# sanweiliti/RoHM

Measured on AMD Instinct MI355X. Metric: denoised 145-frame clips/sec @1000 DDPM steps, higher is better.
Workload: dtype f32

## Files before the change

rohm_amd/csrc/attention_tile.h:

```cpp
#pragma once
#include "common.h"
#include "planes.h"

namespace rohm {

constexpr int AT_S = 144;
constexpr int AT_DH = 128;
constexpr int AT_NB = 9;
constexpr int AT_TILE = AT_S * AT_DH;
constexpr int AT_LDS_FLOATS = 2 * AT_TILE + 512;

#define AT_WAIT_VM(n) __builtin_amdgcn_s_waitcnt(((n) & 15) | (7 << 4) | (15 << 8) | (((n) >> 4) << 14))
#define AT_WAIT_LGKM0() __builtin_amdgcn_s_waitcnt(15 | (7 << 4) | (0 << 8) | (3 << 14))

template <int AUX>
__device__ __forceinline__ void at_dma16(const float* src, float* lds_dst) {
    __builtin_amdgcn_global_load_lds((const __attribute__((address_space(1))) void*)src,
                                     (__attribute__((address_space(3))) void*)lds_dst, 16, 0, AUX);
}

#ifdef AT_TIMELINE
#define AT_TL_PARAM , unsigned long long* __restrict__ tl
#define AT_STAMP(i)                                                                                          \
    do {                                                                                                     \
        if (lane == 0) tl[((size_t)blockIdx.x * NW + wave) * 16 + (i)] = __builtin_amdgcn_s_memtime();     \
    } while (0)
#else
#define AT_TL_PARAM
#define AT_STAMP(i)
#endif

template <int NW, int NPO = 0, int AUX = 0, int NPASS = 1>
__device__ __forceinline__ void attention_item(const float* __restrict__ qkv, float* __restrict__ ctx, int n_head, int item, int q0,
                                               int nq, float* smem, const int tid AT_TL_PARAM) {
    constexpr int OWNED = NW * NPASS;
    constexpr int NQP = (NPASS == 2) ? 72 / NW : ((NW == 8) ? 9 : 10);
    constexpr int NKP = 24 / NW;
    constexpr int NVP = 72 / NW;
    constexpr int NV3 = NVP / 3;
    constexpr int NT = (AT_NB + NW - 1) / NW;
    float* Ks = smem;
    float* Vs = smem + AT_TILE;
    float* dummy = smem + 2 * AT_TILE;
    float* stats = dummy + 256;

    const int lane = tid & 63;
    const int wave = __builtin_amdgcn_readfirstlane(tid >> 6);
    const int li = lane & 15, lg = lane >> 4;

    AT_STAMP(0);
    const bool coop = nq > OWNED;
    const int seq = item / n_head, head = item % n_head;
    const int D = n_head * AT_DH;
    const size_t ldq = (size_t)3 * D;
    const float* qg = qkv + (size_t)seq * AT_S * ldq + head * AT_DH;
    const float* kg = qg + D;
    const float* vg = qg + 2 * D;

    const int half_row = lane >> 5, cphys = lane & 31;
#pragma unroll
    for (int i = 0; i < NQP; ++i) {
        const int lp = i * NW + wave;
        const bool ok = lp < nq * 8;
        const int lr = ok ? 2 * lp + half_row : half_row;
        const float* src = qg + (size_t)(q0 * 16 + lr) * ldq + ((cphys ^ (lr & 15)) << 2);
        at_dma16<AUX>(src, ok ? Vs + lp * 256 : dummy);
    }
    auto issue_k = [&](int G) {
#pragma unroll
        for (int i = 0; i < NKP; ++i) {
            const int piece = 24 * G + i * NW + wave;
            const int row = 2 * piece + half_row;
            at_dma16<AUX>(kg + (size_t)row * ldq + ((cphys ^ (row & 15)) << 2), Ks + piece * 256);
        }
    };
    issue_k(0);
    AT_WAIT_VM(NKP);
    __builtin_amdgcn_s_barrier();
    AT_STAMP(1);

    f32x4 qf[NPASS][8], qc[8];
#pragma unroll
    for (int ks = 0; ks < 8; ++ks) {
#pragma unroll
        for (int ps = 0; ps < NPASS; ++ps)
            qf[ps][ks] = *reinterpret_cast<const f32x4*>(Vs + ((ps * NW + wave) * 16 + li) * AT_DH + (((ks * 4 + lg) ^ li) << 2));
        qc[ks] = *reinterpret_cast<const f32x4*>(Vs + ((coop ? OWNED : 0) * 16 + li) * AT_DH + (((ks * 4 + lg) ^ li) << 2));
    }
    AT_WAIT_LGKM0();
    __builtin_amdgcn_s_barrier();
    auto issue_v = [&](int part) {
#pragma unroll
        for (int i = part * NV3; i < (part + 1) * NV3; ++i) {
            const int piece = i * NW + wave;
            at_dma16<AUX>(vg + (size_t)(2 * piece + half_row) * ldq + (cphys << 2), Vs + piece * 256);
        }
    };
    issue_k(1);
    issue_k(2);

    f32x4 sacc[NPASS][AT_NB];
#pragma unroll
    for (int ps = 0; ps < NPASS; ++ps)
#pragma unroll
        for (int kb = 0; kb < AT_NB; ++kb) sacc[ps][kb] = f32x4{0.f, 0.f, 0.f, 0.f};
#pragma unroll
    for (int G = 0; G < 3; ++G) {
        if (G == 0) {
            AT_WAIT_VM(2 * NKP);
        } else if (G == 1) {
            issue_v(0);
            issue_v(1);
            AT_WAIT_VM(NKP + 2 * NV3);
        } else {
            issue_v(2);
            AT_WAIT_VM(3 * NV3);
        }
        __builtin_amdgcn_s_barrier();
        AT_STAMP(2 + G);
        auto kread = [&](f32x4* kf, int ks) {
#pragma unroll
            for (int c = 0; c < 3; ++c)
                kf[c] = *reinterpret_cast<const f32x4*>(Ks + ((3 * G + c) * 16 + li) * AT_DH + (((ks * 4 + lg) ^ li) << 2));
        };
        f32x4 kf[2][3];
        kread(kf[0], 0);
#pragma unroll
        for (int ks = 0; ks < 8; ++ks) {
#pragma unroll
            for (int c = 0; c < 3; ++c)
                sacc[0][3 * G + c] = __builtin_amdgcn_mfma_f32_16x16x4f32(kf[ks & 1][c][0], qf[0][ks][0], sacc[0][3 * G + c], 0, 0, 0);
            __builtin_amdgcn_sched_barrier(0);
            if (ks + 1 < 8) kread(kf[(ks + 1) & 1], ks + 1);
            __builtin_amdgcn_sched_barrier(0);
#pragma unroll
            for (int j = 1; j < 4; ++j)
#pragma unroll
                for (int c = 0; c < 3; ++c)
                    sacc[0][3 * G + c] = __builtin_amdgcn_mfma_f32_16x16x4f32(kf[ks & 1][c][j], qf[0][ks][j], sacc[0][3 * G + c], 0, 0, 0);
        }
    }
    if constexpr (NPASS == 2) {
#pragma unroll
        for (int G = 0; G < 3; ++G) {
            auto kread = [&](f32x4* kf, int ks) {
#pragma unroll
                for (int c = 0; c < 3; ++c)
                    kf[c] = *reinterpret_cast<const f32x4*>(Ks + ((3 * G + c) * 16 + li) * AT_DH + (((ks * 4 + lg) ^ li) << 2));
            };
            f32x4 kf[2][3];
            kread(kf[0], 0);
#pragma unroll
            for (int ks = 0; ks < 8; ++ks) {
#pragma unroll
                for (int c = 0; c < 3; ++c)
                    sacc[NPASS - 1][3 * G + c] = __builtin_amdgcn_mfma_f32_16x16x4f32(kf[ks & 1][c][0], qf[NPASS - 1][ks][0], sacc[NPASS - 1][3 * G + c], 0, 0, 0);
                __builtin_amdgcn_sched_barrier(0);
                if (ks + 1 < 8) kread(kf[(ks + 1) & 1], ks + 1);
                __builtin_amdgcn_sched_barrier(0);
#pragma unroll
                for (int j = 1; j < 4; ++j)
#pragma unroll
                    for (int c = 0; c < 3; ++c)
                        sacc[NPASS - 1][3 * G + c] = __builtin_amdgcn_mfma_f32_16x16x4f32(kf[ks & 1][c][j], qf[NPASS - 1][ks][j], sacc[NPASS - 1][3 * G + c], 0, 0, 0);
            }
        }
    }
    f32x4 cs[NT];
#pragma unroll
    for (int t = 0; t < NT; ++t) cs[t] = f32x4{0.f, 0.f, 0.f, 0.f};
    if (coop) {
// ... 15 lines not shown
    AT_STAMP(5);
    constexpr float LOG2E = 1.4426950408889634f;
#pragma unroll
    for (int ps = 0; ps < NPASS; ++ps) {
        float mx = sacc[ps][0][0];
#pragma unroll
        for (int kb = 0; kb < AT_NB; ++kb)
#pragma unroll
            for (int r = 0; r < 4; ++r) mx = fmaxf(mx, sacc[ps][kb][r]);
        mx = fmaxf(mx, __shfl_xor(mx, 16));
        mx = fmaxf(mx, __shfl_xor(mx, 32));
        const float mb = mx * LOG2E;
        float sum = 0.f;
#pragma unroll
        for (int kb = 0; kb < AT_NB; ++kb)
#pragma unroll
            for (int r = 0; r < 4; ++r) {
                const float e = __builtin_amdgcn_exp2f(fmaf(sacc[ps][kb][r], LOG2E, -mb));
                sacc[ps][kb][r] = e;
                sum += e;
            }
        sum += __shfl_xor(sum, 16);
        sum += __shfl_xor(sum, 32);
        const float inv = 1.0f / sum;
#pragma unroll
        for (int kb = 0; kb < AT_NB; ++kb)
#pragma unroll
            for (int r = 0; r < 4; ++r) sacc[ps][kb][r] *= inv;
    }
    float c_m = -INFINITY, c_l = 0.f;
    if (coop) {
#pragma unroll
        for (int t = 0; t < NT; ++t)
            if (wave + t * NW < AT_NB)
#pragma unroll
                for (int r = 0; r < 4; ++r) c_m = fmaxf(c_m, cs[t][r]);
        c_m = fmaxf(c_m, __shfl_xor(c_m, 16));
        c_m = fmaxf(c_m, __shfl_xor(c_m, 32));
        const float mb = c_m * LOG2E;
#pragma unroll
        for (int t = 0; t < NT; ++t)
            if (wave + t * NW < AT_NB)
#pragma unroll
                for (int r = 0; r < 4; ++r) {
                    const float e = __builtin_amdgcn_exp2f(fmaf(cs[t][r], LOG2E, -mb));
                    cs[t][r] = e;
                    c_l += e;
                }
        c_l += __shfl_xor(c_l, 16);
        c_l += __shfl_xor(c_l, 32);
    }

    AT_STAMP(6);
    AT_WAIT_VM(0);
    __builtin_amdgcn_s_barrier();
    AT_STAMP(7);

    if (coop) {
        float* part = Ks + wave * (16 * AT_DH);
#pragma unroll
        for (int db = 0; db < 2; ++db) {
            f32x4 oacc[4];
#pragma unroll
            for (int m = 0; m < 4; ++m) oacc[m] = f32x4{0.f, 0.f, 0.f, 0.f};
#pragma unroll
            for (int t = 0; t < NT; ++t) {
                const int kb = wave + t * NW;
                if (kb < AT_NB) {
#pragma unroll
                    for (int j = 0; j < 4; ++j) {
                        const f32x4 vf = *reinterpret_cast<const f32x4*>(Vs + (kb * 16 + lg * 4 + j) * AT_DH + db * 64 + li * 4);
#pragma unroll
                        for (int m = 0; m < 4; ++m)
                            oacc[m] = __builtin_amdgcn_mfma_f32_16x16x4f32(cs[t][j], vf[m], oacc[m], 0, 0, 0);
                    }
                }
            }
#pragma unroll
            for (int r = 0; r < 4; ++r)
                *reinterpret_cast<f32x4*>(part + (lg * 4 + r) * AT_DH + db * 64 + li * 4) =
                    f32x4{oacc[0][r], oacc[1][r], oacc[2][r], oacc[3][r]};
        }
        if (lg == 0) {
            stats[(wave * 16 + li) * 2 + 0] = c_m;
            stats[(wave * 16 + li) * 2 + 1] = c_l;
        }
    }
    AT_STAMP(9);

    {
        auto pv_mfma = [](float pval, float vval, const f32x4& c) {
            if constexpr (NPO == 0) return __builtin_amdgcn_mfma_f32_16x16x4f32(pval, vval, c, 0, 0, 0);
            else return __builtin_amdgcn_mfma_f32_16x16x4f32(vval, pval, c, 0, 0, 0);
        };
#pragma unroll
        for (int ps = 0; ps < NPASS; ++ps) {
        float* out = ctx + ((size_t)seq * AT_S + (q0 + ps * NW + wave) * 16) * D + head * AT_DH;
#pragma unroll
        for (int db = 0; db < 2; ++db) {
            f32x4 oacc[4];
#pragma unroll
            for (int m = 0; m < 4; ++m) oacc[m] = f32x4{0.f, 0.f, 0.f, 0.f};
            auto vread = [&](int st) {
                return *reinterpret_cast<const f32x4*>(Vs + ((st >> 2) * 16 + lg * 4 + (st & 3)) * AT_DH + db * 64 + li * 4);
            };
            f32x4 vf[2][2];
            vf[0][0] = vread(0);
            vf[0][1] = vread(1);
#pragma unroll
            for (int sp = 0; sp < 2 * AT_NB; ++sp) {
                const int st = 2 * sp;
                oacc[0] = pv_mfma(sacc[ps][st >> 2][st & 3], vf[sp & 1][0][0], oacc[0]);
                __builtin_amdgcn_sched_barrier(0);
                if (sp + 1 < 2 * AT_NB) {
                    vf[(sp + 1) & 1][0] = vread(st + 2);
                    vf[(sp + 1) & 1][1] = vread(st + 3);
                }
                __builtin_amdgcn_sched_barrier(0);
#pragma unroll
                for (int m = 1; m < 4; ++m)
                    oacc[m] = pv_mfma(sacc[ps][st >> 2][st & 3], vf[sp & 1][0][m], oacc[m]);
#pragma unroll
                for (int m = 0; m < 4; ++m)
                    oacc[m] = pv_mfma(sacc[ps][(st + 1) >> 2][(st + 1) & 3], vf[sp & 1][1][m], oacc[m]);
            }
            if constexpr (NPO == 0) {
#pragma unroll
                for (int r = 0; r < 4; ++r)
                    *reinterpret_cast<f32x4*>(out + (size_t)(lg * 4 + r) * D + db * 64 + li * 4) =
                        f32x4{oacc[0][r], oacc[1][r], oacc[2][r], oacc[3][r]};
            } else {
                const int row = seq * AT_S + (q0 + ps * NW + wave) * 16 + li;
                const int kg0 = (head * AT_DH + db * 64 + lg * 16) >> 3;
#pragma unroll
                for (int h = 0; h < 2; ++h)
                    plane_store8<(NPO ? NPO : 2)>(reinterpret_cast<char*>(ctx), row, kg0 + h, D / 32,
                                                  f32x4{oacc[0][2 * h], oacc[1][2 * h], oacc[2][2 * h], oacc[3][2 * h]},
                                                  f32x4{oacc[0][2 * h + 1], oacc[1][2 * h + 1], oacc[2][2 * h + 1], oacc[3][2 * h + 1]});
            }
        }
        }
    }
    AT_STAMP(8);
    if (!coop) return;

    AT_WAIT_LGKM0();
    __builtin_amdgcn_s_barrier();
    AT_STAMP(10);
    {
        float* out = ctx + ((size_t)seq * AT_S + (q0 + OWNED) * 16) * D + head * AT_DH;
        for (int u = tid; u < 16 * 32; u += NW * 64) {
            const int q = u >> 5, c4 = u & 31;
            float M = -INFINITY;
#pragma unroll
            for (int w = 0; w < NW; ++w) M = fmaxf(M, stats[(w * 16 + q) * 2]);
            float e[NW], L = 0.f;
#pragma unroll
// ... 24 lines not shown
```

rohm_amd/csrc/encoder_chain.hip:

```cpp
#include <type_traits>
#include "common.h"
#include "gemm_sched.h"
#include "attention_tile.h"

namespace rohm {

typedef float f32x16c __attribute__((ext_vector_type(16)));

namespace chain {

constexpr int BM = 144, BK = kGemmBK, NRB = BM / 16;
constexpr int A_UNITS = BM * 8, A_ITERS = (A_UNITS + 255) / 256;
constexpr int kMaxBN = 384;
constexpr int kZone = 2 * (BM + kMaxBN) * BK;
constexpr int kLdsFloats = kZone + 512 + 4 * BM * 2;
constexpr int kSc1 = 16;

struct PhaseArgs {
    const float* A; int lda;
    const float* W; int ldw;
    float* C; int ldc;
    int K;
    const float* bias;
    const float* R; int ldr;
    const float* gamma; const float* beta; float eps; int ln_dim;
    int qcols; float qscale;
    int S; const float* tab; const float* tab0; int ldtab, ldtab0, tab_by_row;
    int m0, n0;
    float* row_stats; unsigned tag28; int tn, tiles_n;
    unsigned* err; unsigned xcc1; int fault;
};

template <int BN>
__device__ __forceinline__ void prefetch_w(const float* W, int ldw, int n0, float* smem, int tid, int wave_u) {
    constexpr int B_ITERS = BN * 8 / 256;
    float* Bs = smem + 2 * BM * BK;
#pragma unroll
    for (int buf = 0; buf < 2; ++buf)
#pragma unroll
        for (int i = 0; i < B_ITERS; ++i) {
            const int u = tid + i * 256;
            const int row = u >> 3;
            const int slot = (u & 7) ^ ((row >> 1) & 7);
            const float* src = W + (size_t)(n0 + row) * ldw + slot * 4 + buf * BK;
            __builtin_amdgcn_global_load_lds((const __attribute__((address_space(1))) void*)src,
                                             (__attribute__((address_space(3))) void*)(Bs + buf * (BN * BK) + (i * 256 + wave_u) * 4), 16, 0, 0);
        }
}

__device__ __forceinline__ void group_sync(unsigned long long* flags, int tn, int G, unsigned tag, unsigned xcc1, unsigned* err, int tid) {
    asm volatile("s_waitcnt vmcnt(0)" ::: "memory");
    __syncthreads();
    if (tid == 0) {
        flags[tn] = ((unsigned long long)xcc1 << 32) | tag;
        asm volatile("" ::: "memory");
    }
    if (tid < G && tid != tn) {
        for (int it = 0;; ++it) {
            const unsigned long long f = __hip_atomic_load(flags + tid, __ATOMIC_RELAXED, __HIP_MEMORY_SCOPE_AGENT);
            if ((unsigned)f == tag && (f >> 32) != 0ull) {
                if ((unsigned)(f >> 32) != xcc1) __hip_atomic_store(err, 2u, __ATOMIC_RELAXED, __HIP_MEMORY_SCOPE_AGENT);
                break;
            }
            __builtin_amdgcn_s_sleep(1);
            if ((it & 127) == 127 && __hip_atomic_load(err, __ATOMIC_RELAXED, __HIP_MEMORY_SCOPE_AGENT) != 0u) break;
            if (it > (1 << 19)) {
                __hip_atomic_store(err, 1u, __ATOMIC_RELAXED, __HIP_MEMORY_SCOPE_AGENT);
                break;
            }
        }
    }
    __syncthreads();
}

template <int BN, int EPI, bool PREF, bool SC1, bool REFETCH, typename AfterLoop>
__device__ __forceinline__ void gemm_phase(const PhaseArgs& p, float* smem, const int tid, AfterLoop&& after_loop) {
    static_assert(EPI == EPI_BIAS_RES_LN || EPI == EPI_BIAS_GELU || EPI == EPI_QKV || EPI == EPI_EMBED, "chain phases: LN tail, GELU, QKV, embed");
    constexpr int WN = BN / 4;
    constexpr int NCB = WN / 16;
    constexpr int B_ITERS = BN * 8 / 256;
    constexpr int PIECES = A_ITERS + B_ITERS;
    constexpr int AUX = SC1 ? kSc1 : 0;

    float* As = smem;
    float* Bs = smem + 2 * BM * BK;
    float* lds_dummy = smem + kZone;
    float* const zone = lds_dummy + 512;

    const int lane = tid & 63;
    const int wave = tid >> 6;
    const int li = lane & 15, lg = lane >> 4;
    const int wave_u = __builtin_amdgcn_readfirstlane(wave) * 64;
    const int m0 = p.m0, n0 = p.n0;

    const float* a_src[A_ITERS];
#pragma unroll
    for (int i = 0; i < A_ITERS; ++i) {
        const int u = tid + i * 256;
        const int row = (u < A_UNITS) ? (u >> 3) : 0;
        const int slot = (u & 7) ^ ((row >> 1) & 7);
        a_src[i] = p.A + (size_t)(m0 + row) * p.lda + slot * 4;
    }
    const float* b_src[B_ITERS];
#pragma unroll
    for (int i = 0; i < B_ITERS; ++i) {
        const int u = tid + i * 256;
        const int row = u >> 3;
        const int slot = (u & 7) ^ ((row >> 1) & 7);
        b_src[i] = p.W + (size_t)(n0 + row) * p.ldw + slot * 4;
    }
    auto dma_a = [&](int buf, int k0) {
#pragma unroll
        for (int piece = 0; piece < A_ITERS; ++piece) {
            float* dst = As + buf * (BM * BK) + (piece * 256 + wave_u) * 4;
            if (piece == A_ITERS - 1 && A_UNITS % 256 != 0)
                dst = (wave_u < A_UNITS - (A_ITERS - 1) * 256) ? dst : lds_dummy + (wave_u & 64) * 4;
            __builtin_amdgcn_global_load_lds((const __attribute__((address_space(1))) void*)(a_src[piece] + k0),
                                             (__attribute__((address_space(3))) void*)dst, 16, 0, AUX);
        }
    };
    auto dma_b = [&](int buf, int k0) {
#pragma unroll
        for (int i = 0; i < B_ITERS; ++i)
            __builtin_amdgcn_global_load_lds((const __attribute__((address_space(1))) void*)(b_src[i] + k0),
                                             (__attribute__((address_space(3))) void*)(Bs + buf * (BN * BK) + (i * 256 + wave_u) * 4), 16, 0, 0);
    };

    f32x4 acc16[NRB * NCB];
#pragma unroll
    for (int i = 0; i < NRB * NCB; ++i) acc16[i] = f32x4{0.f, 0.f, 0.f, 0.f};
    constexpr int READS = NRB + NCB;
    constexpr int MFMAS = 4 * NRB * NCB;
    struct Frag { f32x4 a[NRB]; f32x4 b[NCB]; };
    Frag f0, f1;
    auto read_frags = [&](Frag& f, int buf, int ks) {
        const float* as = As + buf * (BM * BK);
        const float* bs = Bs + buf * (BN * BK) + wave * WN * BK;
        const int slot = ks * 4 + lg;
#pragma unroll
        for (int c = 0; c < NCB; ++c) f.b[c] = *reinterpret_cast<const f32x4*>(bs + lds_off(c * 16 + li, slot));
#pragma unroll
        for (int r = 0; r < NRB; ++r) f.a[r] = *reinterpret_cast<const f32x4*>(as + lds_off(r * 16 + li, slot));
    };
    auto mma_half = [&](const Frag& f) {
#pragma unroll
        for (int r = 0; r < NRB; ++r)
#pragma unroll
            for (int c = 0; c < NCB; ++c)
#pragma unroll
                for (int j = 0; j < 4; ++j)
                    acc16[r * NCB + c] = __builtin_amdgcn_mfma_f32_16x16x4f32(f.b[c][j], f.a[r][j], acc16[r * NCB + c], 0, 0, 0);
    };

    const int nk = p.K / BK;
    constexpr bool COL_LDS = BN >= 384;
    if constexpr (!PREF) { dma_b(0, 0); dma_b(1, BK); }
    if constexpr (COL_LDS) {
        if (wave == 0) {
#pragma unroll
            for (int h = 0; h < 2; ++h) {
                const int unit = h * 64 + lane;
                const float* src = p.bias + n0 + (unit < BN / 4 ? unit : BN / 4 - 1) * 4;
                __builtin_amdgcn_global_load_lds((const __attribute__((address_space(1))) void*)src,
                                                 (__attribute__((address_space(3))) void*)(zone + h * 256), 16, 0, 0);
            }
        }
    }
    dma_a(0, 0);
    dma_a(1, BK);

    const int nw = n0 + wave * WN;
    struct ColOps { f32x4 bias, g4, b4; };
    constexpr bool RES = (EPI == EPI_BIAS_RES_LN);
    constexpr bool HAS_RES = RES || EPI == EPI_EMBED;
    constexpr bool PEEL = BN <= 256;
    constexpr bool EARLY = PEEL && !COL_LDS;
    const f32x4 zero4 = f32x4{0.f, 0.f, 0.f, 0.f};
    auto load_col = [&](int nb) __attribute__((always_inline)) {
        ColOps o{zero4, zero4, zero4};
        if constexpr (EPI == EPI_EMBED) {  }
        else if constexpr (COL_LDS) o.bias = *reinterpret_cast<const f32x4*>(zone + (nb - n0));
        else o.bias = *reinterpret_cast<const f32x4*>(p.bias + nb);
        if constexpr (RES) {
            o.g4 = *reinterpret_cast<const f32x4*>(p.gamma + nb);
            o.b4 = *reinterpret_cast<const f32x4*>(p.beta + nb);
        }
        return o;
    };
    auto for_units = [&](auto&& fn) __attribute__((always_inline)) {
#pragma unroll
        for (int r = 0; r < NRB; ++r)
#pragma unroll
            for (int c = 0; c < NCB; ++c) fn(c * NRB + r, c, m0 + r * 16 + li, nw + c * 16 + lg * 4, acc16[r * NCB + c]);
    };
    ColOps col[NCB];
    f32x4 res[HAS_RES ? NCB * NRB : 1];
    auto request_ops = [&]() __attribute__((always_inline)) {
#pragma unroll
        for (int c = 0; c < NCB; ++c) col[c] = load_col(nw + c * 16 + lg * 4);
        if constexpr (RES)
            for_units([&](int i, int, int m, int nb, f32x4) __attribute__((always_inline)) {
                res[i] = *reinterpret_cast<const f32x4*>(p.R + (size_t)m * p.ldr + nb);
            });
        if constexpr (EPI == EPI_EMBED)
            for_units([&](int i, int, int m, int nb, f32x4) __attribute__((always_inline)) {
                const int bidx = m / p.S, tok = m % p.S;
                const float* tp = (tok == 0) ? p.tab0 + (size_t)bidx * p.ldtab0 + nb : p.tab + (size_t)(p.tab_by_row ? m : tok) * p.ldtab + nb;
                res[i] = *reinterpret_cast<const f32x4*>(tp);
            });
    };

    asm volatile("s_waitcnt vmcnt(%0)" ::"n"(A_ITERS) : "memory");
    __syncthreads();
    read_frags(f0, 0, 0);
    constexpr int NG = READS;
    constexpr int MF = (MFMAS + NG - 1) / NG;
    auto chunk = [&](int kc, auto last_tag, auto dma_tag) __attribute__((always_inline)) {
        constexpr bool LAST = decltype(last_tag)::value;
        constexpr bool DMA = decltype(dma_tag)::value;
        const int buf = kc & 1;
        if constexpr (LAST && EARLY) request_ops();
        read_frags(f1, buf, 1);
        mma_half(f0);
        SchedGroups<0, NG, MF, READS, 0, 0>::run();
        __builtin_amdgcn_sched_barrier(0);
        if constexpr (!LAST) {
            asm volatile("s_waitcnt vmcnt(0)" ::: "memory");
            __syncthreads();
            __builtin_amdgcn_sched_barrier(0);
            if constexpr (DMA) {
                const int kn = ((kc + 2 < nk) ? (kc + 2) : (nk - 1)) * BK;
                dma_a(buf, kn);
                dma_b(buf, kn);
            }
// ... 93 lines not shown
                    }
                }
                bool ok = true, same_xcd = true;
#pragma unroll
                for (int k = 0; k < 8; ++k) {
                    mk[k] = 0.f; qk[k] = 0.f;
                    if (k >= tiles_n) continue;
                    if (k == tn) { mk[k] = a; qk[k] = b; continue; }
                    const unsigned tl = (unsigned)(lo[k] >> 32), th = (unsigned)(hi[k] >> 32);
                    ok = ok && (tl >> 4) == ep28 && (th >> 4) == ep28 && (tl & 15u) != 0u && (th & 15u) != 0u;
                    same_xcd = same_xcd && (tl & 15u) == xcc1 && (th & 15u) == xcc1;
                    mk[k] = __uint_as_float((unsigned)lo[k]);
                    qk[k] = __uint_as_float((unsigned)hi[k]);
                }
                if (ok) {
                    if (!same_xcd) __hip_atomic_store(p.err, 2u, __ATOMIC_RELAXED, __HIP_MEMORY_SCOPE_AGENT);
                    break;
                }
                __builtin_amdgcn_s_sleep(1);
                if ((it & 127) == 127 && __hip_atomic_load(p.err, __ATOMIC_RELAXED, __HIP_MEMORY_SCOPE_AGENT) != 0u) break;
                if (it > (1 << 19)) {
                    __hip_atomic_store(p.err, 1u, __ATOMIC_RELAXED, __HIP_MEMORY_SCOPE_AGENT);
                    break;
                }
            }
            constexpr float kT = (float)BN;
            if (tiles_n > 1) {
                merge(mk[0], qk[0], mk[1], qk[1], kT, mk[0], qk[0]);
                if (tiles_n > 2) merge(mk[2], qk[2], mk[3], qk[3], kT, mk[2], qk[2]);
                if (tiles_n > 4) { merge(mk[4], qk[4], mk[5], qk[5], kT, mk[4], qk[4]); merge(mk[6], qk[6], mk[7], qk[7], kT, mk[6], qk[6]); }
            }
            if (tiles_n > 2) {
                merge(mk[0], qk[0], mk[2], qk[2], 2.0f * kT, mk[0], qk[0]);
                if (tiles_n > 4) merge(mk[4], qk[4], mk[6], qk[6], 2.0f * kT, mk[4], qk[4]);
            }
            if (tiles_n > 4) merge(mk[0], qk[0], mk[4], qk[4], 4.0f * kT, mk[0], qk[0]);
            const float mu = mk[0];
            const float var = qk[0] / (float)p.ln_dim;
            *reinterpret_cast<f32x2*>(part + tid * 2) = f32x2{mu, 1.0f / sqrtf(var + p.eps)};
        }
        __syncthreads();
#pragma unroll
        for (int r = 0; r < NRB; ++r) {
            const f32x2 mrv = *reinterpret_cast<const f32x2*>(part + (r * 16 + li) * 2);
#pragma unroll
            for (int c = 0; c < NCB; ++c) {
                const f32x4 a = acc16[r * NCB + c];
                f32x4 v;
#pragma unroll
                for (int q = 0; q < 4; ++q) v[q] = (a[q] - mrv[0]) * mrv[1] * col[c].g4[q] + col[c].b4[q];
                *reinterpret_cast<f32x4*>(p.C + (size_t)(m0 + r * 16 + li) * p.ldc + nw + c * 16 + lg * 4) = v;
            }
        }
    } else if constexpr (EPI == EPI_EMBED) {
        for_units([&](int i, int, int m, int nb, f32x4 a) __attribute__((always_inline)) {
            const int tok = m % p.S;
            f32x4 v;
#pragma unroll
            for (int q = 0; q < 4; ++q) v[q] = (tok == 0 ? 0.f : a[q]) + res[i][q];
            *reinterpret_cast<f32x4*>(p.C + (size_t)m * p.ldc + nb) = v;
        });
    } else {
        for_units([&](int, int cg, int m, int nb, f32x4 a) __attribute__((always_inline)) {
            f32x4 v;
#pragma unroll
            for (int q = 0; q < 4; ++q) v[q] = a[q] + col[cg].bias[q];
            if constexpr (EPI == EPI_BIAS_GELU) {
#pragma unroll
                for (int q = 0; q < 4; ++q) v[q] = gelu_erf(v[q]);
            }
            if constexpr (EPI == EPI_QKV) {
                if (nb < p.qcols) {
#pragma unroll
                    for (int q = 0; q < 4; ++q) v[q] *= p.qscale;
                }
            }
            *reinterpret_cast<f32x4*>(p.C + (size_t)m * p.ldc + nb) = v;
        });
    }
}

template <int G>
__device__ __forceinline__ void head_tail_phase(const StackParams& p, const int g, const int tn, float* smem, const int tid) {
    constexpr int NC_OWN = 16 / G;
    constexpr int NW = NC_OWN * 16 + 16;
    constexpr int NRMAX = (G == 4) ? 9 : 5;
    constexpr int W_UNITS = NW * 8, W_ITERS = (W_UNITS + 255) / 256;
    constexpr int PIECES = A_ITERS + W_ITERS;
    constexpr int kBuf = (BM + NW) * BK;
    static_assert(3 * kBuf <= kZone, "head phase: staging buffers overrun the zone");
    float* lds_dummy = smem + kZone;
    const int lane = tid & 63, li = lane & 15, lg = lane >> 4;
    const int wave = __builtin_amdgcn_readfirstlane(tid >> 6);
    const int wave_u = wave * 64;
    const int D = p.D, m0 = g * BM;
    int c_loc, r0, nr, e;
    if constexpr (G == 4) { c_loc = wave; r0 = 0; nr = 9; e = tn * 4 + wave; }
    else { c_loc = wave >> 1; r0 = (wave & 1) ? 5 : 0; nr = (wave & 1) ? 4 : 5; e = (wave & 1) ? tn * 2 + (wave >> 1) : 99; }
    const bool has_e = e < NRB;

    const float* a_src[A_ITERS];
#pragma unroll
    for (int i = 0; i < A_ITERS; ++i) {
        const int u = tid + i * 256;
        const int row = (u < A_UNITS) ? (u >> 3) : 0;
        const int slot = (u & 7) ^ ((row >> 1) & 7);
// ... 171 lines not shown
    const int tid = threadIdx.x;
    const int wave_u = __builtin_amdgcn_readfirstlane(tid >> 6) * 64;
    const int x = blockIdx.x % kNumXCD, j = blockIdx.x / kNumXCD;
    const int g = (j / G) * kNumXCD + x, tn = j % G;
    if (g >= p.tiles_m) return;
    const unsigned xcc1 = 1u + (unsigned)__builtin_amdgcn_s_getreg((3 << 11) | 20);
    const unsigned ep = p.epoch + 64u * *p.xln_pass;
    if (tid == 0) p.xln_xcc[g * 8 + tn] = xcc1;
    unsigned long long* const flags = p.flags + (size_t)g * 9 * 5 * 8;

    PhaseArgs a{};
    a.m0 = g * BM; a.err = p.xln_err; a.xcc1 = xcc1; a.tn = tn; a.tiles_n = G;
    a.row_stats = p.xln_stats + ((size_t)g * G * BM) * 4;
    a.eps = p.ln_eps; a.ln_dim = p.D;

    a.A = p.ctx; a.lda = p.D; a.W = p.out_w; a.ldw = p.D; a.C = p.y; a.ldc = p.D; a.K = p.D; a.bias = p.out_b;
    a.R = p.h; a.ldr = p.D; a.gamma = p.n1_w; a.beta = p.n1_b; a.n0 = tn * BNL; a.tag28 = ep & 0x0fffffffu; a.fault = p.fault & 1;
    gemm_phase<BNL, EPI_BIAS_RES_LN, false, false, G == 8>(a, smem, tid, [&]() { prefetch_w<BNF>(p.l1_w, p.D, tn * BNF, smem, tid, wave_u); });
    group_sync(flags, tn, G, ep, xcc1, p.xln_err, tid);

    a.A = p.y; a.lda = p.D; a.W = p.l1_w; a.ldw = p.D; a.C = p.ff; a.ldc = p.F; a.K = p.D; a.bias = p.l1_b; a.n0 = tn * BNF;
    gemm_phase<BNF, EPI_BIAS_GELU, true, true, G == 8>(a, smem, tid, [&]() { prefetch_w<BNL>(p.l2_w, p.F, tn * BNL, smem, tid, wave_u); });
    group_sync(flags + 8, tn, G, ep, xcc1, p.xln_err, tid);

    a.A = p.ff; a.lda = p.F; a.W = p.l2_w; a.ldw = p.F; a.C = p.h; a.ldc = p.D; a.K = p.F; a.bias = p.l2_b;
    a.R = p.y; a.ldr = p.D; a.gamma = p.n2_w; a.beta = p.n2_b; a.n0 = tn * BNL; a.tag28 = (ep + 1u) & 0x0fffffffu; a.fault = (p.fault >> 1) & 1;
    gemm_phase<BNL, EPI_BIAS_RES_LN, true, true, G == 8>(a, smem, tid, [&]() { if (p.qkv) prefetch_w<BNQ>(p.in_w, p.D, tn * BNQ, smem, tid, wave_u); });
    if (p.qkv == nullptr) return;
    group_sync(flags + 16, tn, G, ep, xcc1, p.xln_err, tid);

    a.A = p.h; a.lda = p.D; a.W = p.in_w; a.ldw = p.D; a.C = p.qkv; a.ldc = 3 * p.D; a.K = p.D; a.bias = p.in_b; a.n0 = tn * BNQ;
    a.qcols = p.D; a.qscale = p.qscale;
    gemm_phase<BNQ, EPI_QKV, true, true, G == 8>(a, smem, tid, []() {});
}

template <int G>
__global__ __launch_bounds__(256) void encoder_stack_kernel(StackParams p) {
    using namespace chain;
    constexpr int BNL = 512 / G, BNF = 1024 / G, BNQ = 1536 / G;
    extern __shared__ __attribute__((aligned(16))) float smem[];
    const int tid0 = threadIdx.x;
    const int x = blockIdx.x % kNumXCD, j = blockIdx.x / kNumXCD;
    const int g = (j / G) * kNumXCD + x, tn = j % G;
    if (g >= p.tiles_m) return;
    const unsigned xcc1 = 1u + (unsigned)__builtin_amdgcn_s_getreg((3 << 11) | 20);
    const unsigned ep = p.epoch + 64u * (*p.xln_pass + p.pass_add);
    if (tid0 == 0) p.xln_xcc[g * 8 + tn] = xcc1;

    PhaseArgs a{};
    a.m0 = g * BM; a.err = p.xln_err; a.xcc1 = xcc1; a.tn = tn; a.tiles_n = G;
    a.row_stats = p.xln_stats + ((size_t)g * G * BM) * 4;
    a.eps = p.ln_eps; a.ln_dim = p.D;
    a.qcols = p.D; a.qscale = p.qscale;
    unsigned long long* const tl = p.timeline ? p.timeline + (size_t)blockIdx.x * kStackTimelineLayers * kStackTimelineStamps : nullptr;
    auto stamp = [&](int layer, int k) __attribute__((always_inline)) {
        if (tl != nullptr && threadIdx.x == 0) tl[layer * kStackTimelineStamps + k] = __builtin_amdgcn_s_memrealtime();
    };
    {
    int tid = tid0;
    asm volatile("" : "+v"(tid));
    const int wave_u = __builtin_amdgcn_readfirstlane(tid >> 6) * 64;
    unsigned long long* const fl = p.flags + ((size_t)g * 9 + 8) * 5 * 8;
    a.A = p.apack; a.lda = p.lda_pack; a.W = p.w_embed; a.ldw = p.ldw_embed; a.C = p.h; a.ldc = p.D; a.K = p.k_embed; a.n0 = tn * BNL;
    a.S = p.S; a.tab = p.tab; a.tab0 = p.tab0; a.ldtab = p.ldtab; a.ldtab0 = p.ldtab0; a.tab_by_row = p.tab_by_row;
    stamp(8, 0);
    gemm_phase<BNL, EPI_EMBED, false, false, G == 8>(a, smem, tid, [&]() { prefetch_w<BNQ>(p.layer[0].in_w, p.D, tn * BNQ, smem, tid, wave_u); });
    stamp(8, 1);
    group_sync(fl, tn, G, ep, xcc1, p.xln_err, tid);
    stamp(8, 2);
    a.A = p.h; a.lda = p.D; a.W = p.layer[0].in_w; a.ldw = p.D; a.C = p.qkv; a.ldc = 3 * p.D; a.K = p.D; a.bias = p.layer[0].in_b;
    a.n0 = tn * BNQ;
    gemm_phase<BNQ, EPI_QKV, true, true, G == 8>(a, smem, tid, []() {});
    stamp(8, 3);
    group_sync(fl + 8, tn, G, ep, xcc1, p.xln_err, tid);
    stamp(8, 4);
    }
#pragma unroll 1
    for (int l = 0; l < p.L; ++l) {
        int tid = tid0;
        asm volatile("" : "+v"(tid));
        const int wave_u = __builtin_amdgcn_readfirstlane(tid >> 6) * 64;
        const StackLayerW& w = p.layer[l];
        unsigned long long* const fl = p.flags + ((size_t)g * 9 + l) * 5 * 8;
        stamp(l, 0);
        if (l > 0) group_sync(fl, tn, G, ep, xcc1, p.xln_err, tid);
        stamp(l, 1);
        if constexpr (G == 4) attention_item<4, 0, kSc1, 2>(p.qkv, p.ctx, p.n_head, g * p.n_head + tn, 0, AT_NB, smem, tid);
        else attention_item<4, 0, kSc1, 1>(p.qkv, p.ctx, p.n_head, g * p.n_head + (tn >> 1), (tn & 1) ? 5 : 0, (tn & 1) ? 4 : 5, smem, tid);
        stamp(l, 2);
        group_sync(fl + 8, tn, G, ep, xcc1, p.xln_err, tid);
        stamp(l, 3);

        a.A = p.ctx; a.lda = p.D; a.W = w.out_w; a.ldw = p.D; a.C = p.y; a.ldc = p.D; a.K = p.D; a.bias = w.out_b;
        a.R = p.h; a.ldr = p.D; a.gamma = w.n1_w; a.beta = w.n1_b; a.n0 = tn * BNL; a.tag28 = (ep + 4u * l) & 0x0fffffffu;
        a.fault = (l == 0) ? (p.fault & 1) : 0;
        gemm_phase<BNL, EPI_BIAS_RES_LN, false, true, G == 8>(a, smem, tid, [&]() { prefetch_w<BNF>(w.l1_w, p.D, tn * BNF, smem, tid, wave_u); });
        stamp(l, 4);
        group_sync(fl + 16, tn, G, ep, xcc1, p.xln_err, tid);
        stamp(l, 5);

        a.A = p.y; a.lda = p.D; a.W = w.l1_w; a.ldw = p.D; a.C = p.ff; a.ldc = p.F; a.K = p.D; a.bias = w.l1_b; a.n0 = tn * BNF;
        gemm_phase<BNF, EPI_BIAS_GELU, true, true, G == 8>(a, smem, tid, [&]() { prefetch_w<BNL>(w.l2_w, p.F, tn * BNL, smem, tid, wave_u); });
        stamp(l, 6);
        group_sync(fl + 24, tn, G, ep, xcc1, p.xln_err, tid);
        stamp(l, 7);

        const bool more = l + 1 < p.L;
        a.A = p.ff; a.lda = p.F; a.W = w.l2_w; a.ldw = p.F; a.C = p.h; a.ldc = p.D; a.K = p.F; a.bias = w.l2_b;
        a.R = p.y; a.ldr = p.D; a.gamma = w.n2_w; a.beta = w.n2_b; a.n0 = tn * BNL; a.tag28 = (ep + 4u * l + 1u) & 0x0fffffffu;
        a.fault = (l == 0) ? ((p.fault >> 1) & 1) : 0;
        gemm_phase<BNL, EPI_BIAS_RES_LN, true, true, G == 8>(a, smem, tid, [&]() { if (more) prefetch_w<BNQ>(p.layer[l + 1].in_w, p.D, tn * BNQ, smem, tid, wave_u); });
        stamp(l, 8);
        if (!more) {
            if (p.tail) {
                group_sync(fl + 32, tn, G, ep, xcc1, p.xln_err, tid);
                stamp(l, 9);
                head_tail_phase<G>(p, g, tn, smem, tid);
                stamp(l, 10);
                if (p.t_pass_ctr != nullptr && blockIdx.x == 0 && threadIdx.x == 0) p.t_pass_ctr[1] = p.pass_add + 1u;
            }
            break;
        }
        group_sync(fl + 32, tn, G, ep, xcc1, p.xln_err, tid);
        stamp(l, 9);

        a.A = p.h; a.lda = p.D; a.W = p.layer[l + 1].in_w; a.ldw = p.D; a.C = p.qkv; a.ldc = 3 * p.D; a.K = p.D; a.bias = p.layer[l + 1].in_b;
        a.n0 = tn * BNQ;
        gemm_phase<BNQ, EPI_QKV, true, true, G == 8>(a, smem, tid, []() {});
        stamp(l, 10);
    }
}

int launch_encoder_stack(const StackParams& p, hipStream_t s) {
    const int G = encoder_chain_parts(p.M, p.D, p.F);
    ROHM_ARG_CHECK(G != 0 && p.n_head == 4 && p.L >= 1 && p.L <= 8, "encoder_stack: shape (M %d, D %d, F %d, %d heads, %d layers) has no stack form",
                   p.M, p.D, p.F, p.n_head, p.L);
    ROHM_ARG_CHECK(p.h && p.y && p.ff && p.qkv && p.ctx && p.xln_stats && p.xln_err && p.xln_pass && p.xln_xcc && p.flags, "encoder_stack: null operand");
    ROHM_ARG_CHECK(p.apack && p.w_embed && p.tab && p.tab0 && p.S == chain::BM && p.k_embed >= 2 * chain::BK && p.k_embed % chain::BK == 0 &&
                       p.lda_pack % 4 == 0 && p.ldw_embed % 4 == 0 && p.ldtab % 4 == 0 && p.ldtab0 % 4 == 0,
                   "encoder_stack: bad operands of the leading embed phase");
    StackParams q = p;
    q.tiles_m = p.M / chain::BM;
    const int groups8 = (q.tiles_m + kNumXCD - 1) / kNumXCD * kNumXCD;
    ROHM_ARG_CHECK(!p.tail || (p.D == 512 && p.t_out_w && p.t_out_b && p.t_x && p.t_cond && p.t_C - p.t_traj == 272 &&
                               p.t_T == chain::BM - 1 && p.t_traj > 0 && (!p.t_apack || p.t_lda >= p.t_C)),
                   "encoder_stack: the closing head / update / pack phase needs whole 144-token clips, d_model 512 and 272 predicted channels");
    constexpr int kFloats = AT_LDS_FLOATS > chain::kLdsFloats ? AT_LDS_FLOATS : chain::kLdsFloats;
    const size_t lds = (size_t)kFloats * sizeof(float);
    static bool attr_set[64][2] = {};
    int dev = 0;
    ROHM_HIP_CHECK(hipGetDevice(&dev));
    if (dev < 64 && !attr_set[dev][G == 8]) {
        if (G == 4) ROHM_HIP_CHECK(hipFuncSetAttribute(reinterpret_cast<const void*>(&encoder_stack_kernel<4>), hipFuncAttributeMaxDynamicSharedMemorySize, (int)lds));
        else ROHM_HIP_CHECK(hipFuncSetAttribute(reinterpret_cast<const void*>(&encoder_stack_kernel<8>), hipFuncAttributeMaxDynamicSharedMemorySize, (int)lds));
        attr_set[dev][G == 8] = true;
    }
    const double MM = (double)p.M, D = p.D, F = p.F, L = p.L;
    const double flops = L * (4.0 * 144.0 * 128.0 * MM * p.n_head + 2.0 * MM * (D * D + 2.0 * D * F)) + L * 2.0 * MM * 3.0 * D * D +
                         2.0 * MM * D * p.k_embed;
    const double bytes = 4.0 * (L * (MM * (3.0 * D + D + 4.0 * D + 2.0 * F + D) + D * D + 2.0 * D * F) + (L - 1.0) * (MM * 3.0 * D + 3.0 * D * D));
    const double tail_flops = p.tail ? 2.0 * MM * D * (p.t_C - p.t_traj) : 0.0;
    prof::Scope ps(p.tail ? "gemm_stack_tail" : "gemm_stack", flops + tail_flops, bytes, s);
    if (G == 4) hipLaunchKernelGGL(encoder_stack_kernel<4>, dim3(groups8 * 4), dim3(256), lds, s, q);
    else hipLaunchKernelGGL(encoder_stack_kernel<8>, dim3(groups8 * 8), dim3(256), lds, s, q);
    ROHM_LAUNCH_CHECK();
    return ROHM_OK;
}

int encoder_chain_parts(int M, int D, int F) {
    if (D != 512 || F != 1024 || M <= 0 || M % chain::BM != 0) return 0;
    const int tm = M / chain::BM;
    return tm >= 48 ? 4 : 8;
}

bool encoder_chain_pays(int B) {
    if (B <= 0) return false;
    if (B < 48) return B > 24 && B <= 32;
    if (B <= 64) return true;
    const int wgs = (B + kNumXCD - 1) / kNumXCD * kNumXCD * 4, rounds = (wgs + 255) / 256;
    return 4 * B * 100 >= 93 * rounds * 256;
}

// ... 32 lines not shown
```

Baseline: 22.79.

## Fuse QKV projection with attention via head-aligned tiles kept resident in LDS

For the 4-block group configuration, the QKV GEMM now tiles one head's q|k|v columns per block through a head-row permutation of the weights and bias. Its epilogue writes K and V straight into the attention LDS layout and hands Q fragments to the attention code in registers. Attention then runs without reloading Q/K/V from global memory and without the inter-block group sync between the QKV GEMM and attention. This removes a global round trip and a cross-block barrier per layer, at the cost of a swizzled V layout, extra registers for the Q fragments, and tighter LDS sharing.

```diff
diff --git a/rohm_amd/csrc/attention_tile.h b/rohm_amd/csrc/attention_tile.h
--- a/rohm_amd/csrc/attention_tile.h
+++ b/rohm_amd/csrc/attention_tile.h
@@ -30,9 +30,12 @@
 #define AT_STAMP(i)
 #endif
 
-template <int NW, int NPO = 0, int AUX = 0, int NPASS = 1>
+template <int NPASS>
+struct AtQFrags { f32x4 f[NPASS][8]; f32x4 c[8]; };
+
+template <int NW, int NPO = 0, int AUX = 0, int NPASS = 1, bool RESIDENT = false>
 __device__ __forceinline__ void attention_item(const float* __restrict__ qkv, float* __restrict__ ctx, int n_head, int item, int q0,
-                                               int nq, float* smem, const int tid AT_TL_PARAM) {
+                                               int nq, float* smem, const int tid AT_TL_PARAM, const AtQFrags<NPASS>* qin = nullptr) {
     constexpr int OWNED = NW * NPASS;
     constexpr int NQP = (NPASS == 2) ? 72 / NW : ((NW == 8) ? 9 : 10);
     constexpr int NKP = 24 / NW;
@@ -56,16 +59,13 @@
     const float* qg = qkv + (size_t)seq * AT_S * ldq + head * AT_DH;
     const float* kg = qg + D;
     const float* vg = qg + 2 * D;
+    auto vaddr = [&](int key, int db) __attribute__((always_inline)) {
+        if constexpr (RESIDENT) return Vs + key * AT_DH + (((db * 16 + li) ^ (key & 15)) << 2);
+        else return Vs + key * AT_DH + db * 64 + li * 4;
+    };
 
     const int half_row = lane >> 5, cphys = lane & 31;
-#pragma unroll
-    for (int i = 0; i < NQP; ++i) {
-        const int lp = i * NW + wave;
-        const bool ok = lp < nq * 8;
-        const int lr = ok ? 2 * lp + half_row : half_row;
-        const float* src = qg + (size_t)(q0 * 16 + lr) * ldq + ((cphys ^ (lr & 15)) << 2);
-        at_dma16<AUX>(src, ok ? Vs + lp * 256 : dummy);
-    }
+    f32x4 qf[NPASS][8], qc[8];
     auto issue_k = [&](int G) {
 #pragma unroll
         for (int i = 0; i < NKP; ++i) {
@@ -74,21 +74,6 @@
             at_dma16<AUX>(kg + (size_t)row * ldq + ((cphys ^ (row & 15)) << 2), Ks + piece * 256);
         }
     };
-    issue_k(0);
-    AT_WAIT_VM(NKP);
-    __builtin_amdgcn_s_barrier();
-    AT_STAMP(1);
-
-    f32x4 qf[NPASS][8], qc[8];
-#pragma unroll
-    for (int ks = 0; ks < 8; ++ks) {
-#pragma unroll
-        for (int ps = 0; ps < NPASS; ++ps)
-            qf[ps][ks] = *reinterpret_cast<const f32x4*>(Vs + ((ps * NW + wave) * 16 + li) * AT_DH + (((ks * 4 + lg) ^ li) << 2));
-        qc[ks] = *reinterpret_cast<const f32x4*>(Vs + ((coop ? OWNED : 0) * 16 + li) * AT_DH + (((ks * 4 + lg) ^ li) << 2));
-    }
-    AT_WAIT_LGKM0();
-    __builtin_amdgcn_s_barrier();
     auto issue_v = [&](int part) {
 #pragma unroll
         for (int i = part * NV3; i < (part + 1) * NV3; ++i) {
@@ -96,8 +81,39 @@
             at_dma16<AUX>(vg + (size_t)(2 * piece + half_row) * ldq + (cphys << 2), Vs + piece * 256);
         }
     };
-    issue_k(1);
-    issue_k(2);
+    if constexpr (RESIDENT) {
+#pragma unroll
+        for (int ks = 0; ks < 8; ++ks) {
+#pragma unroll
+            for (int ps = 0; ps < NPASS; ++ps) qf[ps][ks] = qin->f[ps][ks];
+            qc[ks] = qin->c[ks];
+        }
+    } else {
+#pragma unroll
+        for (int i = 0; i < NQP; ++i) {
+            const int lp = i * NW + wave;
+            const bool ok = lp < nq * 8;
+            const int lr = ok ? 2 * lp + half_row : half_row;
+            const float* src = qg + (size_t)(q0 * 16 + lr) * ldq + ((cphys ^ (lr & 15)) << 2);
+            at_dma16<AUX>(src, ok ? Vs + lp * 256 : dummy);
+        }
+        issue_k(0);
+        AT_WAIT_VM(NKP);
+        __builtin_amdgcn_s_barrier();
+        AT_STAMP(1);
+
+#pragma unroll
+        for (int ks = 0; ks < 8; ++ks) {
+#pragma unroll
+            for (int ps = 0; ps < NPASS; ++ps)
+                qf[ps][ks] = *reinterpret_cast<const f32x4*>(Vs + ((ps * NW + wave) * 16 + li) * AT_DH + (((ks * 4 + lg) ^ li) << 2));
+            qc[ks] = *reinterpret_cast<const f32x4*>(Vs + ((coop ? OWNED : 0) * 16 + li) * AT_DH + (((ks * 4 + lg) ^ li) << 2));
+        }
+        AT_WAIT_LGKM0();
+        __builtin_amdgcn_s_barrier();
+        issue_k(1);
+        issue_k(2);
+    }
 
     f32x4 sacc[NPASS][AT_NB];
 #pragma unroll
@@ -106,17 +122,19 @@
         for (int kb = 0; kb < AT_NB; ++kb) sacc[ps][kb] = f32x4{0.f, 0.f, 0.f, 0.f};
 #pragma unroll
     for (int G = 0; G < 3; ++G) {
-        if (G == 0) {
-            AT_WAIT_VM(2 * NKP);
-        } else if (G == 1) {
-            issue_v(0);
-            issue_v(1);
-            AT_WAIT_VM(NKP + 2 * NV3);
-        } else {
-            issue_v(2);
-            AT_WAIT_VM(3 * NV3);
-        }
-        __builtin_amdgcn_s_barrier();
+        if constexpr (!RESIDENT) {
+            if (G == 0) {
+                AT_WAIT_VM(2 * NKP);
+            } else if (G == 1) {
+                issue_v(0);
+                issue_v(1);
+                AT_WAIT_VM(NKP + 2 * NV3);
+            } else {
+                issue_v(2);
+                AT_WAIT_VM(3 * NV3);
+            }
+            __builtin_amdgcn_s_barrier();
+        }
         AT_STAMP(2 + G);
         auto kread = [&](f32x4* kf, int ks) {
 #pragma unroll
@@ -238,7 +256,7 @@
     }
 
     AT_STAMP(6);
-    AT_WAIT_VM(0);
+    if constexpr (!RESIDENT) AT_WAIT_VM(0);
     __builtin_amdgcn_s_barrier();
     AT_STAMP(7);
 
@@ -255,7 +273,7 @@
                 if (kb < AT_NB) {
 #pragma unroll
                     for (int j = 0; j < 4; ++j) {
-                        const f32x4 vf = *reinterpret_cast<const f32x4*>(Vs + (kb * 16 + lg * 4 + j) * AT_DH + db * 64 + li * 4);
+                        const f32x4 vf = *reinterpret_cast<const f32x4*>(vaddr(kb * 16 + lg * 4 + j, db));
 #pragma unroll
                         for (int m = 0; m < 4; ++m)
                             oacc[m] = __builtin_amdgcn_mfma_f32_16x16x4f32(cs[t][j], vf[m], oacc[m], 0, 0, 0);
@@ -288,7 +306,7 @@
 #pragma unroll
             for (int m = 0; m < 4; ++m) oacc[m] = f32x4{0.f, 0.f, 0.f, 0.f};
             auto vread = [&](int st) {
-                return *reinterpret_cast<const f32x4*>(Vs + ((st >> 2) * 16 + lg * 4 + (st & 3)) * AT_DH + db * 64 + li * 4);
+                return *reinterpret_cast<const f32x4*>(vaddr((st >> 2) * 16 + lg * 4 + (st & 3), db));
             };
             f32x4 vf[2][2];
             vf[0][0] = vread(0);
diff --git a/rohm_amd/csrc/encoder_chain.hip b/rohm_amd/csrc/encoder_chain.hip
--- a/rohm_amd/csrc/encoder_chain.hip
+++ b/rohm_amd/csrc/encoder_chain.hip
@@ -31,7 +31,9 @@
     unsigned* err; unsigned xcc1; int fault;
 };
 
-template <int BN>
+__device__ __forceinline__ int head_row(int n0, int t) { return ((t % 96) >> 5) * 512 + n0 + (t / 96) * 32 + (t & 31); }
+
+template <int BN, bool HEAD = false>
 __device__ __forceinline__ void prefetch_w(const float* W, int ldw, int n0, float* smem, int tid, int wave_u) {
     constexpr int B_ITERS = BN * 8 / 256;
     float* Bs = smem + 2 * BM * BK;
@@ -42,7 +44,7 @@
             const int u = tid + i * 256;
             const int row = u >> 3;
             const int slot = (u & 7) ^ ((row >> 1) & 7);
-            const float* src = W + (size_t)(n0 + row) * ldw + slot * 4 + buf * BK;
+            const float* src = W + (size_t)(HEAD ? head_row(n0, row) : n0 + row) * ldw + slot * 4 + buf * BK;
             __builtin_amdgcn_global_load_lds((const __attribute__((address_space(1))) void*)src,
                                              (__attribute__((address_space(3))) void*)(Bs + buf * (BN * BK) + (i * 256 + wave_u) * 4), 16, 0, 0);
         }
@@ -73,9 +75,11 @@
     __syncthreads();
 }
 
-template <int BN, int EPI, bool PREF, bool SC1, bool REFETCH, typename AfterLoop>
-__device__ __forceinline__ void gemm_phase(const PhaseArgs& p, float* smem, const int tid, AfterLoop&& after_loop) {
+template <int BN, int EPI, bool PREF, bool SC1, bool REFETCH, bool HEAD = false, typename AfterLoop>
+__device__ __forceinline__ void gemm_phase(const PhaseArgs& p, float* smem, const int tid, AfterLoop&& after_loop,
+                                           AtQFrags<2>* q_out = nullptr) {
     static_assert(EPI == EPI_BIAS_RES_LN || EPI == EPI_BIAS_GELU || EPI == EPI_QKV || EPI == EPI_EMBED, "chain phases: LN tail, GELU, QKV, embed");
+    static_assert(!HEAD || (EPI == EPI_QKV && BN == 3 * AT_DH), "the head-aligned tile is one head's q | k | v");
     constexpr int WN = BN / 4;
     constexpr int NCB = WN / 16;
     constexpr int B_ITERS = BN * 8 / 256;
@@ -86,6 +90,8 @@
     float* Bs = smem + 2 * BM * BK;
     float* lds_dummy = smem + kZone;
     float* const zone = lds_dummy + 512;
+    float* const colrow = HEAD ? smem + 2 * AT_TILE : zone;
+    static_assert(!HEAD || 2 * AT_TILE + 512 <= AT_LDS_FLOATS, "head-aligned tile: the bias row overruns the stack's LDS");
 
     const int lane = tid & 63;
     const int wave = tid >> 6;
@@ -107,7 +113,7 @@
         const int u = tid + i * 256;
         const int row = u >> 3;
         const int slot = (u & 7) ^ ((row >> 1) & 7);
-        b_src[i] = p.W + (size_t)(n0 + row) * p.ldw + slot * 4;
+        b_src[i] = p.W + (size_t)(HEAD ? head_row(n0, row) : n0 + row) * p.ldw + slot * 4;
     }
     auto dma_a = [&](int buf, int k0) {
 #pragma unroll
@@ -160,9 +166,10 @@
 #pragma unroll
             for (int h = 0; h < 2; ++h) {
                 const int unit = h * 64 + lane;
-                const float* src = p.bias + n0 + (unit < BN / 4 ? unit : BN / 4 - 1) * 4;
+                const int t = (unit < BN / 4 ? unit : BN / 4 - 1) * 4;
+                const float* src = HEAD ? p.bias + head_row(n0, t) : p.bias + n0 + t;
                 __builtin_amdgcn_global_load_lds((const __attribute__((address_space(1))) void*)src,
-                                                 (__attribute__((address_space(3))) void*)(zone + h * 256), 16, 0, 0);
+                                                 (__attribute__((address_space(3))) void*)(colrow + h * 256), 16, 0, 0);
             }
         }
     }
@@ -179,7 +186,7 @@
     auto load_col = [&](int nb) __attribute__((always_inline)) {
         ColOps o{zero4, zero4, zero4};
         if constexpr (EPI == EPI_EMBED) {  }
-        else if constexpr (COL_LDS) o.bias = *reinterpret_cast<const f32x4*>(zone + (nb - n0));
+        else if constexpr (COL_LDS) o.bias = *reinterpret_cast<const f32x4*>(colrow + (nb - n0));
         else o.bias = *reinterpret_cast<const f32x4*>(p.bias + nb);
         if constexpr (RES) {
             o.g4 = *reinterpret_cast<const f32x4*>(p.gamma + nb);
@@ -379,6 +386,36 @@
                 *reinterpret_cast<f32x4*>(p.C + (size_t)(m0 + r * 16 + li) * p.ldc + nw + c * 16 + lg * 4) = v;
             }
         }
+    } else if constexpr (HEAD) {
+        float* const Ks = smem;
+        float* const Vs = smem + AT_TILE;
+        auto put = [&](float* img, int c) __attribute__((always_inline)) {
+            const int u = wave * 8 + (c & 1) * 4 + lg;
+#pragma unroll
+            for (int r = 0; r < NRB; ++r) {
+                const f32x4 a = acc16[r * NCB + c];
+                f32x4 v;
+#pragma unroll
+                for (int q = 0; q < 4; ++q) v[q] = a[q] + col[c].bias[q];
+                if (c < 2) {
+#pragma unroll
+                    for (int q = 0; q < 4; ++q) v[q] *= p.qscale;
+                }
+                *reinterpret_cast<f32x4*>(img + (r * 16 + li) * AT_DH + ((u ^ li) << 2)) = v;
+            }
+        };
+        put(Vs, 0); put(Vs, 1);
+        put(Ks, 2); put(Ks, 3);
+        __syncthreads();
+#pragma unroll
+        for (int ks = 0; ks < 8; ++ks) {
+            const int sw = ((ks * 4 + lg) ^ li) << 2;
+#pragma unroll
+            for (int ps = 0; ps < 2; ++ps) q_out->f[ps][ks] = *reinterpret_cast<const f32x4*>(Vs + ((ps * 4 + wave) * 16 + li) * AT_DH + sw);
+            q_out->c[ks] = *reinterpret_cast<const f32x4*>(Vs + (8 * 16 + li) * AT_DH + sw);
+        }
+        __syncthreads();
+        put(Vs, 4); put(Vs, 5);
     } else if constexpr (EPI == EPI_EMBED) {
         for_units([&](int i, int, int m, int nb, f32x4 a) __attribute__((always_inline)) {
             const int tok = m % p.S;
@@ -656,9 +693,27 @@
     a.row_stats = p.xln_stats + ((size_t)g * G * BM) * 4;
     a.eps = p.ln_eps; a.ln_dim = p.D;
     a.qcols = p.D; a.qscale = p.qscale;
+    constexpr bool HEAD = G == 4;
+    auto n0q = [&]() __attribute__((always_inline)) { return HEAD ? tn * AT_DH : tn * BNQ; };
+    AtQFrags<2> qh;
     unsigned long long* const tl = p.timeline ? p.timeline + (size_t)blockIdx.x * kStackTimelineLayers * kStackTimelineStamps : nullptr;
     auto stamp = [&](int layer, int k) __attribute__((always_inline)) {
         if (tl != nullptr && threadIdx.x == 0) tl[layer * kStackTimelineStamps + k] = __builtin_amdgcn_s_memrealtime();
+    };
+    auto attend = [&](int l, int tid) __attribute__((always_inline)) {
+        unsigned long long* const fl = p.flags + ((size_t)g * 9 + l) * 5 * 8;
+        stamp(l, 0);
+        if (l > 0) {
+            if constexpr (HEAD) __syncthreads();
+            else group_sync(fl, tn, G, ep, xcc1, p.xln_err, tid);
+        }
+        stamp(l, 1);
+        if constexpr (HEAD)
+            attention_item<4, 0, kSc1, 2, true>(p.qkv, p.ctx, p.n_head, g * p.n_head + tn, 0, AT_NB, smem, tid, &qh);
+        else attention_item<4, 0, kSc1, 1>(p.qkv, p.ctx, p.n_head, g * p.n_head + (tn >> 1), (tn & 1) ? 5 : 0, (tn & 1) ? 4 : 5, smem, tid);
+        stamp(l, 2);
+        group_sync(fl + 8, tn, G, ep, xcc1, p.xln_err, tid);
+        stamp(l, 3);
     };
     {
     int tid = tid0;
@@ -668,16 +723,18 @@
     a.A = p.apack; a.lda = p.lda_pack; a.W = p.w_embed; a.ldw = p.ldw_embed; a.C = p.h; a.ldc = p.D; a.K = p.k_embed; a.n0 = tn * BNL;
     a.S = p.S; a.tab = p.tab; a.tab0 = p.tab0; a.ldtab = p.ldtab; a.ldtab0 = p.ldtab0; a.tab_by_row = p.tab_by_row;
     stamp(8, 0);
-    gemm_phase<BNL, EPI_EMBED, false, false, G == 8>(a, smem, tid, [&]() { prefetch_w<BNQ>(p.layer[0].in_w, p.D, tn * BNQ, smem, tid, wave_u); });
+    gemm_phase<BNL, EPI_EMBED, false, false, G == 8>(a, smem, tid, [&]() { prefetch_w<BNQ, HEAD>(p.layer[0].in_w, p.D, n0q(), smem, tid, wave_u); });
     stamp(8, 1);
     group_sync(fl, tn, G, ep, xcc1, p.xln_err, tid);
     stamp(8, 2);
     a.A = p.h; a.lda = p.D; a.W = p.layer[0].in_w; a.ldw = p.D; a.C = p.qkv; a.ldc = 3 * p.D; a.K = p.D; a.bias = p.layer[0].in_b;
-    a.n0 = tn * BNQ;
-    gemm_phase<BNQ, EPI_QKV, true, true, G == 8>(a, smem, tid, []() {});
+    a.n0 = n0q();
+    gemm_phase<BNQ, EPI_QKV, true, true, G == 8, HEAD>(a, smem, tid, []() {}, &qh);
     stamp(8, 3);
-    group_sync(fl + 8, tn, G, ep, xcc1, p.xln_err, tid);
+    if constexpr (HEAD) __syncthreads();
+    else group_sync(fl + 8, tn, G, ep, xcc1, p.xln_err, tid);
     stamp(8, 4);
+    if constexpr (HEAD) attend(0, tid);
     }
 #pragma unroll 1
     for (int l = 0; l < p.L; ++l) {
@@ -686,14 +743,7 @@
         const int wave_u = __builtin_amdgcn_readfirstlane(tid >> 6) * 64;
         const StackLayerW& w = p.layer[l];
         unsigned long long* const fl = p.flags + ((size_t)g * 9 + l) * 5 * 8;
-        stamp(l, 0);
-        if (l > 0) group_sync(fl, tn, G, ep, xcc1, p.xln_err, tid);
-        stamp(l, 1);
-        if constexpr (G == 4) attention_item<4, 0, kSc1, 2>(p.qkv, p.ctx, p.n_head, g * p.n_head + tn, 0, AT_NB, smem, tid);
-        else attention_item<4, 0, kSc1, 1>(p.qkv, p.ctx, p.n_head, g * p.n_head + (tn >> 1), (tn & 1) ? 5 : 0, (tn & 1) ? 4 : 5, smem, tid);
-        stamp(l, 2);
-        group_sync(fl + 8, tn, G, ep, xcc1, p.xln_err, tid);
-        stamp(l, 3);
+        if constexpr (!HEAD) attend(l, tid);
 
         a.A = p.ctx; a.lda = p.D; a.W = w.out_w; a.ldw = p.D; a.C = p.y; a.ldc = p.D; a.K = p.D; a.bias = w.out_b;
         a.R = p.h; a.ldr = p.D; a.gamma = w.n1_w; a.beta = w.n1_b; a.n0 = tn * BNL; a.tag28 = (ep + 4u * l) & 0x0fffffffu;
@@ -713,7 +763,7 @@
         a.A = p.ff; a.lda = p.F; a.W = w.l2_w; a.ldw = p.F; a.C = p.h; a.ldc = p.D; a.K = p.F; a.bias = w.l2_b;
         a.R = p.y; a.ldr = p.D; a.gamma = w.n2_w; a.beta = w.n2_b; a.n0 = tn * BNL; a.tag28 = (ep + 4u * l + 1u) & 0x0fffffffu;
         a.fault = (l == 0) ? ((p.fault >> 1) & 1) : 0;
-        gemm_phase<BNL, EPI_BIAS_RES_LN, true, true, G == 8>(a, smem, tid, [&]() { if (more) prefetch_w<BNQ>(p.layer[l + 1].in_w, p.D, tn * BNQ, smem, tid, wave_u); });
+        gemm_phase<BNL, EPI_BIAS_RES_LN, true, true, G == 8>(a, smem, tid, [&]() { if (more) prefetch_w<BNQ, HEAD>(p.layer[l + 1].in_w, p.D, n0q(), smem, tid, wave_u); });
         stamp(l, 8);
         if (!more) {
             if (p.tail) {
@@ -729,9 +779,10 @@
         stamp(l, 9);
 
         a.A = p.h; a.lda = p.D; a.W = p.layer[l + 1].in_w; a.ldw = p.D; a.C = p.qkv; a.ldc = 3 * p.D; a.K = p.D; a.bias = p.layer[l + 1].in_b;
-        a.n0 = tn * BNQ;
-        gemm_phase<BNQ, EPI_QKV, true, true, G == 8>(a, smem, tid, []() {});
+        a.n0 = n0q();
+        gemm_phase<BNQ, EPI_QKV, true, true, G == 8, HEAD>(a, smem, tid, []() {}, &qh);
         stamp(l, 10);
+        if constexpr (HEAD) attend(l + 1, tid);
     }
 }
 
```

Result: faster. 23.41 (median of 6 runs) (+2.7%).
